# j-wilson/GPflowPILCO

Hardware: AMD Instinct MI355X
Metric: moment_matched_rollout_step_elements_per_sec (higher is better)
Workload: dtype f32; 1 GPU; C3 (BASELINE configs[2]): N=2000 d=8 D=8 H=40 fp32 drift moment-match step / closed rollout; recipe=baseline: BASELINE.md recipe: lengthscales log-U[0.3,3], GP-prior targets, fresh mu~U[0,1]^d / Sigm~; N=2000, d=8, D=8, H=40, B_per_gpu=256, B_total=256, B_this_rank=256, parallelism=dp1 over B (weak), recipe=baseline, steps_requested=418, diag_pairs=f64, offdiag_pairs=f32

## Files before the change

### gpflowpilco_amd/csrc/mm_common.h

```cpp
#pragma once
#include <stddef.h>
#include <stdint.h>
#include "../../include/gpflowpilco_mm.h"

static inline size_t mm_align_up(size_t x, size_t a) { return (x + a - 1) / a * a; }
static inline int mm_round_up_int(int x, int a) { return (x + a - 1) / a * a; }
static inline size_t mm_elem_size(int dtype) { return dtype == MM_F64 ? 8 : 4; }

#define MM_ISTAGE_NO_ROUTE (1 << 20)
#define MM_ISTAGE_ROUTE (1 << 21)
#define MM_ISTAGE_NO_M56 (1 << 22)
#define MM_ISTAGE_OLD_OFFDIAG (1 << 23)

static inline int mm_num_pairs(int L, int flags) {
  return (flags & MM_FULL_OUTPUT_COV) ? L * (L + 1) / 2 : L;
}

static inline int mm_moment_deg(int d) { return d <= 8 ? 4 : 2; }
static inline long long mm_binom(int n, int k) {
  if (k < 0 || k > n) return 0;
  long long r = 1;
  for (int i = 1; i <= k; ++i) r = r * (n - k + i) / i;
  return r;
}
static inline int mm_mono_count(int n, int d) { return (int)mm_binom(d + n - 1, n); }
static inline int mm_mono_offset(int n, int d) { int o = 0; for (int m = 0; m < n; ++m) o += mm_mono_count(m, d); return o; }
static inline size_t mm_rank_table_entries(int d) {
  const int dk = d <= 8 ? 8 : 32, deg = mm_moment_deg(d);
  size_t n = 0, p = 1;
  for (int k = 1; k <= deg; ++k) { p *= dk; n += p; }
  return n;
}
static inline int mm_moment_cols(int d) { return mm_round_up_int(mm_mono_offset(mm_moment_deg(d) + 1, d), 16); }
static inline int mm_moment56_off5(int d) { return d <= 8 ? mm_round_up_int(mm_mono_count(4, d), 128) : 0; }
static inline int mm_moment56_off6(int d) { return d <= 8 ? mm_moment56_off5(d) + mm_round_up_int(mm_mono_count(5, d), 128) : 0; }
static inline int mm_moment56_cols(int d) { return d <= 8 ? mm_moment56_off6(d) + mm_round_up_int(mm_mono_count(6, d), 128) : 0; }
struct MMTab56 { int ins[6], last[6], n_i16, mult2, mult3, n_f32; size_t bytes; };
static inline MMTab56 mm_tab56(int d) {
  MMTab56 t;
  int o = 0;
  for (int m = 0; m < 6; ++m) { t.ins[m] = o; o += mm_mono_count(m, d) * 8; }
  for (int k = 0; k < 6; ++k) { t.last[k] = o; o += mm_mono_count(k, d); }
  t.n_i16 = mm_round_up_int(o, 8);
  t.mult2 = 0; t.mult3 = mm_mono_count(2, d); t.n_f32 = mm_mono_count(2, d) + mm_mono_count(3, d);
  t.bytes = (size_t)t.n_i16 * 2 + (size_t)t.n_f32 * 4;
  return t;
}

struct MMModelLayout {
  int Mp, Kz, nd8, KMp;
  size_t Z64;
  size_t Zt64;
  size_t zbar;
  size_t ls2;
  size_t var;
  size_t meanc;
  size_t beta64;
  size_t Zc64;
  size_t Zc;
  size_t Zs3;
  size_t Zm;
  size_t zmax2;
  size_t rtab;
  size_t Zq2;
  size_t Zm56;
  size_t tab56;
  size_t perm;
  size_t skey;
  size_t zt2;
  size_t Cm;
  size_t total;
};
#define MM_SORT_MIN_M 256

static inline MMModelLayout mm_model_layout(int L, int M, int d, int dtype, int with_C) {
  MMModelLayout o;
  const size_t es = mm_elem_size(dtype), A = 256;
  o.Mp = mm_round_up_int(M, MM_M_ALIGN);
  o.Kz = mm_round_up_int(d, 2);
  o.nd8 = (d + 7) / 8;
  o.KMp = mm_moment_cols(d);
  size_t off = 0;
  o.Z64 = off;    off = mm_align_up(off + (size_t)L * M * d * 8, A);
  o.Zt64 = off;   off = mm_align_up(off + (size_t)L * d * o.Mp * 8, A);
  o.zbar = off;   off = mm_align_up(off + (size_t)L * d * 8, A);
  o.ls2 = off;    off = mm_align_up(off + (size_t)L * d * 8, A);
  o.var = off;    off = mm_align_up(off + (size_t)L * 8, A);
  o.meanc = off;  off = mm_align_up(off + (size_t)L * 8, A);
  o.beta64 = off; off = mm_align_up(off + (size_t)L * M * 8, A);
  o.Zc64 = off;   off = mm_align_up(off + (size_t)L * o.Mp * o.Kz * 8, A);
  o.Zc = o.Zc64;
  if (dtype != MM_F64) { o.Zc = off; off = mm_align_up(off + (size_t)L * o.Mp * o.Kz * es, A); }
  o.Zs3 = off;
  if (dtype != MM_F64) off = mm_align_up(off + (size_t)L * o.Mp * 24 * o.nd8 * 2, A);
  o.Zm = off;
// ... 173 lines not shown
```

### gpflowpilco_amd/csrc/mm_moments.hip

```cpp
#include <hip/hip_runtime.h>
#include <math.h>
#include "mm_common.h"
#include "mm_mono.h"

typedef double f64x4m __attribute__((ext_vector_type(4)));

#define MM_GEMM_RB 64
#define MM_GEMM_NB 128
#define MM_GEMM_KB 32
#define MM_GEMM_AS 34
#define MM_GEMM_BS 144

__device__ __forceinline__ void mm_decode_pair_m(int p, int L, int& a, int& a2) {
  int r = p - L, i = 0;
  while (r >= L - 1 - i) { r -= L - 1 - i; ++i; }
  a = i; a2 = i + 1 + r;
}

__global__ __launch_bounds__(256) __attribute__((amdgpu_waves_per_eu(2, 2))) void k_wmom_gemm(const double* __restrict__ whR, const double* __restrict__ whC,
                                                      const double* __restrict__ Zm, int KMp, int L, int Mp, int B, int Po,
                                                      int nrb, int ncb, int nwork, int col_deg3,
                                                      const unsigned int* __restrict__ amaxc, const double* __restrict__ zmax2,
                                                      const int* __restrict__ gperm, double* __restrict__ mom) {
  const int orig = blockIdx.x;
// ... 235 lines not shown
    const int dsz = 1 << (LB * n);
    const int offn = n == 1 ? off1 : n == 2 ? off2 : n == 3 ? off3 : off4;
    const short* rtn = rtab + (((1 << (LB * n)) - DK) / (DK - 1));
    for (int idx = tid; idx < dsz; idx += 256) {
      const int r = rtn[idx];
      T[MM_PADI(idx)] = r >= 0 ? qh[offn + r] : 0.0;
    }
    __syncthreads();
    for (int t = 0; t < n; ++t) {
      const int sh = LB * t, nfib = dsz >> LB;
      for (int f = tid; f < nfib; f += 256) {
        const int lo = f & ((1 << sh) - 1), hi = f >> sh;
        const int base = (hi << (sh + LB)) + lo;
        double v[DK];
#pragma unroll
        for (int l = 0; l < DK; ++l) v[l] = T[MM_PADI(base + (l << sh))];
        if constexpr (DK == 8) {
#pragma unroll
          for (int k = 0; k < 8; ++k) {
            double s = 0.0;
#pragma unroll
            for (int l = 0; l < 8; ++l) s = fma(Gr[k * 8 + l], v[l], s);
            T[MM_PADI(base + (k << sh))] = s;
          }
        } else {
#pragma unroll 2
          for (int k = 0; k < DK; ++k) {
            double s = 0.0;
#pragma unroll
            for (int l = 0; l < DK; ++l) s = fma(Gs[k * DK + l], v[l], s);
            T[MM_PADI(base + (k << sh))] = s;
          }
        }
      }
      __syncthreads();
    }
    double* cur = T;
    double* oth = U;
    int ksz = dsz;
    double sign_binom = 1.0;
    for (int k = n; k >= 0; --k) {
      const int offk = k == 0 ? 0 : k == 1 ? off1 : k == 2 ? off2 : k == 3 ? off3 : off4;
      double part = 0.0;
      const short* rtk = rtab + (k ? (((1 << (LB * k)) - DK) / (DK - 1)) : 0);
      for (int idx = tid; idx < ksz; idx += 256) {
        const int r = k ? rtk[idx] : 0;
        if (r >= 0) part = fma(cur[MM_PADI(idx)], nh[offk + r], part);
      }
      total = fma(an * sign_binom, part, total);
      if (k == 0) break;
      const int nsz = ksz >> LB;
      for (int idx = tid; idx < nsz; idx += 256) {
        double s = 0.0;
#pragma unroll
        for (int l = 0; l < DK; ++l) s = fma(cur[MM_PADI(l * nsz + idx)], dmu[l], s);
        oth[MM_PADI(idx)] = s;
      }
      __syncthreads();
      double* tsw = cur; cur = oth; oth = tsw;
      ksz = nsz;
      sign_binom = -sign_binom * (double)k / (double)(n - k + 1);
    }
    __syncthreads();
  }
  const double tot = mm_block_sum256m(total, red);
  if (tid == 0) s12[(size_t)b * Po + po] = tot + nh[0] * qh[0];
#undef MM_PADI
}

int mm_launch_wmom_full(const char* packed, const MMModelLayout& ml, char* ws, const MMWorkspaceLayout& wl,
                        int B, int L, int d, hipStream_t stream) {
  const int nrb = ((L - 1) * B + MM_GEMM_RB - 1) / MM_GEMM_RB, ncb = (ml.KMp + MM_GEMM_NB - 1) / MM_GEMM_NB;
  const long long nwork_ll = (long long)L * ncb * MM_MOM_SPLIT * nrb;
  if (nwork_ll <= 0 || nwork_ll > 0x7fffffffLL) return MM_E_DIM;
  hipLaunchKernelGGL(k_wmom_gemm, dim3((int)nwork_ll), dim3(256), 0, stream, (const double*)(ws + wl.whR),
                     (const double*)(ws + wl.whC), (const double*)(packed + ml.Zm), ml.KMp, L, wl.Mp, B, wl.Po, nrb, ncb,
                     (int)nwork_ll, 0x7fffffff , (const unsigned int*)nullptr, (const double*)(packed + ml.zmax2),
                     (const int*)nullptr, (double*)(ws + wl.mom));
  hipError_t e = hipGetLastError();
  return e == hipSuccess ? 0 : (int)e;
}

int mm_launch_moments56(const char* packed, const MMModelLayout& ml, char* ws, const MMWorkspaceLayout& wl,
                        int B, int L, int d, int allow, hipStream_t stream);

int mm_launch_moments(const char* packed, const MMModelLayout& ml, char* ws, const MMWorkspaceLayout& wl,
                      int B, int L, int d, const void* mu_f32, int flags, hipStream_t stream) {
  const double* Zm = (const double*)(packed + ml.Zm);
  double* mom = (double*)(ws + wl.mom);
  const int deg = mm_moment_deg(d) >= 4 ? 3 : mm_moment_deg(d);
  const int ncol_fwd = mm_mono_offset(deg + 1, d);
  const int nrb = ((L - 1) * B + MM_GEMM_RB - 1) / MM_GEMM_RB, ncb = (ncol_fwd + MM_GEMM_NB - 1) / MM_GEMM_NB;
  const long long nwork_ll = (long long)L * ncb * MM_MOM_SPLIT * nrb;
  if (nwork_ll <= 0 || nwork_ll > 0x7fffffffLL) return MM_E_DIM;
  const int nwork = (int)nwork_ll;
  const int allow = (flags & (MM_FORCE_WORST_TIER | MM_ISTAGE_NO_M56)) ? 0 : 1;
  const int col_deg3 = mm_mono_offset(3, d);
  const bool some = allow && mm_moment_deg(d) >= 4;
  if (some) {
    hipLaunchKernelGGL(k_wmom_perm, dim3(L), dim3(1024), 0, stream, (const unsigned int*)(ws + wl.amaxc),
                       (const double*)(packed + ml.zmax2), L, B, wl.Po, (int*)(ws + wl.gperm));
    hipError_t ep = hipGetLastError();
    if (ep != hipSuccess) return (int)ep;
  }
  hipLaunchKernelGGL(k_wmom_gemm, dim3(nwork), dim3(256), 0, stream, (const double*)(ws + wl.whR),
                     (const double*)(ws + wl.whC), Zm, ml.KMp, L, wl.Mp, B, wl.Po, nrb, ncb, nwork, col_deg3,
                     some ? (const unsigned int*)(ws + wl.amaxc) : (const unsigned int*)nullptr,
                     (const double*)(packed + ml.zmax2), some ? (const int*)(ws + wl.gperm) : (const int*)nullptr, mom);
  hipError_t e = hipGetLastError();
  if (e != hipSuccess) return (int)e;
  const int off1 = mm_mono_offset(1, d), off2 = mm_mono_offset(2, d), off3 = mm_mono_offset(3, d), off4 = mm_mono_offset(4, d);
#define MM_SPOLY(DK_, LB_)                                                                                                       \
  do {                                                                                                                          \
    const int dn_ = 1 << (LB_ * deg);                                                                                           \
    const int up_ = dn_ >> LB_;                                                                                                 \
    const size_t shm_ = (size_t)(dn_ + (dn_ >> 5) + up_ + (up_ >> 5) + 2 * ml.KMp + DK_ * DK_ + DK_ + 8) * sizeof(double);      \
    hipLaunchKernelGGL((k_spoly<DK_, LB_>), dim3(wl.Po, B), dim3(256), shm_, stream, (const double*)mom, ml.KMp,                \
                       (const double*)(ws + wl.pairmat), (const double*)(packed + ml.zbar), (const double*)(packed + ml.zmax2), \
                       (const unsigned int*)(ws + wl.amax), (const unsigned int*)(ws + wl.amaxc), (const float*)mu_f32, L, d, wl.P, deg, allow, off1, off2, off3, off4, \
                       (const short*)(packed + ml.rtab),                                                                        \
                       (double)MM_C6_C0, (double)MM_C6_C1, (double*)(ws + wl.s12));                                             \
  } while (0)
  if (d <= 8) MM_SPOLY(8, 3); else MM_SPOLY(32, 5);
#undef MM_SPOLY
  e = hipGetLastError();
  if (e != hipSuccess) return (int)e;
  if (flags & MM_ISTAGE_NO_M56) {
    if (mm_moment56_cols(d) <= 0 || wl.Po <= 0) return 0;
    const hipError_t em = hipMemsetAsync(ws + wl.s56, 0xFF, (size_t)B * wl.Po * sizeof(double), stream);
    if (em != hipSuccess) return (int)em;
    const hipError_t es = hipMemsetAsync(ws + wl.estS, 0, (size_t)B * wl.Po * sizeof(float), stream);
    return es == hipSuccess ? 0 : (int)es;
  }
  return mm_launch_moments56(packed, ml, ws, wl, B, L, d, some ? 1 : 0, stream);
}

__global__ void k_offdiag_stats(const unsigned int* __restrict__ amax, const double* __restrict__ zmax2,
                                const unsigned char* __restrict__ gflag, int ng, int L, int Po, int n,
                                int32_t* __restrict__ out) {
  const int idx = blockIdx.x * blockDim.x + threadIdx.x;
  bool c = false, in = false, part = false;
  int groups = 0;
  if (idx < n) {
    int a, a2;
    mm_decode_pair_m(L + idx % Po, L, a, a2);
    const float b2 = mm_collapse_bound2(amax[idx], zmax2[a2]);
    c = b2 <= MM_COLLAPSE_BOUND2;
    in = b2 <= MM_INSIDE_BOUND2;
    part = !c && mm_item_collapsed(amax[n + idx]);
    for (int g = 0; g < ng; ++g) groups += gflag[(size_t)idx * ng + g] ? 1 : 0;
  }
  const unsigned long long m = __ballot(c), mi = __ballot(in), mp = __ballot(part);
  if ((threadIdx.x & 63) == 0 && m) atomicAdd(out, (int)__popcll(m));
  if ((threadIdx.x & 63) == 0 && mi) atomicAdd(out + 2, (int)__popcll(mi));
  if ((threadIdx.x & 63) == 0 && mp) atomicAdd(out + 4, (int)__popcll(mp));
#pragma unroll
  for (int off = 32; off > 0; off >>= 1) groups += __shfl_down(groups, off, 64);
  if ((threadIdx.x & 63) == 0 && groups) atomicAdd(out + 5, groups);
  if (idx == 0) out[1] = n;
}

extern "C" int mm_offdiag_stats(const void* packed, size_t packed_bytes, int L, int M, int d, int dtype, int B, int flags,
                                const void* workspace, size_t workspace_bytes, int32_t* out, void* stream) {
  if (!packed || !workspace || !out || L <= 0 || M <= 0 || d <= 0 || d > MM_DMAX || B <= 0) return MM_E_ARG;
  const MMModelLayout ml = mm_model_layout(L, M, d, dtype, 1);
  const MMWorkspaceLayout wl = mm_workspace_layout(B, L, M, d, dtype, flags);
  if (packed_bytes < ml.Cm || workspace_bytes < wl.total) return MM_E_WORKSPACE;
  hipStream_t s = (hipStream_t)stream;
  hipError_t e = hipMemsetAsync(out, 0, 6 * sizeof(int32_t), s);
  if (e != hipSuccess) return (int)e;
  if (dtype == MM_F32 && wl.Po > 0) {
    e = hipMemcpyAsync(out + 3, (const char*)workspace + wl.rcount + 4, sizeof(int32_t), hipMemcpyDeviceToDevice, s);
    if (e != hipSuccess) return (int)e;
  }
  if (dtype != MM_F32 || wl.Po == 0 || mm_moment_deg(d) < 4 || (flags & MM_FORCE_WORST_TIER)) return 0;
  const int n = B * wl.Po;
  hipLaunchKernelGGL(k_offdiag_stats, dim3((n + 255) / 256), dim3(256), 0, s, (const unsigned int*)((const char*)workspace + wl.amax),
                     (const double*)((const char*)packed + ml.zmax2), (const unsigned char*)((const char*)workspace + wl.gflag),
                     wl.Mp / MM_GROUP_ROWS, L, wl.Po, n, out);
  e = hipGetLastError();
  return e == hipSuccess ? 0 : (int)e;
}
```

### gpflowpilco_amd/csrc/mm_moments6.hip

```cpp
#include <hip/hip_runtime.h>
#include <math.h>
#include "mm_common.h"
#include "mm_mono.h"
#include "mm_f32_tile.h"
#include <atomic>
#include <type_traits>

__device__ __forceinline__ void mm6_decode_pair_o(int lp, int L, int& a, int& a2) {
  int r = lp, i = 0;
  while (r >= L - 1 - i) { r -= L - 1 - i; ++i; }
  a = i; a2 = i + 1 + r;
}

__global__ __launch_bounds__(256) void k_pack_zm56(char* packed, MMModelLayout lay, int L, int M, int d, int N56p,
                                                   const double* __restrict__ Z) {
  const int c = blockIdx.x, a = blockIdx.y, tid = threadIdx.x;
  const int n4 = mm_binom_i(d + 3, 4), n5 = mm_binom_i(d + 4, 5), n6 = mm_binom_i(d + 5, 6);
  const int off5 = ((n4 + 127) / 128) * 128;
  const int off6 = off5 + ((n5 + 127) / 128) * 128;
  const double* zbar = (const double*)(packed + lay.zbar) + (size_t)a * d;
  unsigned short* oh = (unsigned short*)(packed + lay.Zm56) + (((size_t)a * 2 + 0) * N56p + c) * lay.Mp;
  unsigned short* om = (unsigned short*)(packed + lay.Zm56) + (((size_t)a * 2 + 1) * N56p + c) * lay.Mp;
  int n = 0, k[6] = {0, 0, 0, 0, 0, 0};
  if (c < n4) { n = 4; mm_mono_unrank(c, 4, k); }
// ... 186 lines not shown
#endif
template <int K, bool TRANSG, int MODE, int NC = MM6_NC, int NW = MM6_WAVES>
__device__ __forceinline__ void mm6_step(const float* __restrict__ Tin, int nJin, int nI, float* __restrict__ Tout, int nJp,
                                         const short* __restrict__ ins, int d, const float (&G)[64], const float* __restrict__ multJ,
                                         int xs, float& acc, int wave, int lane) {
  const int chunks = (nJp + 64 * NC - 1) / (64 * NC);
  auto dots = [&](auto i0c, const float (&v)[NC][8], float (&s)[NC][8]) __attribute__((always_inline)) {
    constexpr int I0 = decltype(i0c)::value;
#pragma unroll
    for (int q = 0; q < NC; ++q)
#pragma unroll
      for (int i = I0; i < 8; ++i) s[q][i] = G[0 * 8 + i] * v[q][0];
#pragma unroll
    for (int j = 1; j < 8; ++j)
#pragma unroll
      for (int q = 0; q < NC; ++q)
#pragma unroll
        for (int i = I0; i < 8; ++i) s[q][i] = fmaf(G[j * 8 + i], v[q][j], s[q][i]);
  };
  auto body = [&](int I, int t, const int (&Jp)[NC], const bool (&jv)[NC], const int (&off)[NC][8], const float (&mj)[NC]) __attribute__((always_inline)) {
    const float* tin = Tin + I * nJin;
    float v[NC][8], s[NC][8];
#pragma unroll
    for (int q = 0; q < NC; ++q)
#pragma unroll
      for (int j = 0; j < 8; ++j) v[q][j] = tin[off[q][j]];
    if (t < 4) dots(std::integral_constant<int, 0>{}, v, s);
    else if (t < 6) dots(std::integral_constant<int, 4>{}, v, s);
    else dots(std::integral_constant<int, 6>{}, v, s);
#pragma unroll
    for (int i = 0; i < 8; ++i) {
      if (i >= t && i < d) {
        const int orow = I + mm_binom_i(i + K, K + 1);
        float m3 = 1.0f;
        if constexpr (MODE == 1 && K == 2) {
          const int a = I - ((t * (t + 1)) >> 1);
          m3 = a == t ? (i == t ? 1.0f : 3.0f) : (i == t ? 3.0f : 6.0f);
        } else if constexpr (MODE == 1 && K == 1) {
          m3 = i == t ? 1.0f : 2.0f;
        }
#pragma unroll
        for (int q = 0; q < NC; ++q) {
          if constexpr (MODE == 0) { if (jv[q]) Tout[orow * nJp + Jp[q]] = s[q][i]; }
          else if constexpr (MODE == 1) { if (jv[q]) Tout[orow * xs + Jp[q]] = (m3 * mj[q]) * s[q][i]; }
          else { if (jv[q]) acc = fmaf(s[q][i], Tout[Jp[q] * xs + orow], acc); }
        }
      }
    }
  };
  const int nunit = chunks * nI;
  const float rnI = 1.0f / (float)nI;
  int cprev = -1, off[NC][8], Jc[NC];
  bool jv[NC];
  float mj[NC];
#pragma unroll
  for (int q = 0; q < NC; ++q) { Jc[q] = 0; jv[q] = false; mj[q] = 0.0f; }
  for (int u = wave; u < nunit; u += NW) {
    int c = K == 0 ? u : (int)(((float)u + 0.5f) * rnI);
    c = __builtin_amdgcn_readfirstlane(c);
    const int I = K == 0 ? 0 : __builtin_amdgcn_readfirstlane(u - c * nI);
    if (c != cprev) {
      cprev = c;
#pragma unroll
      for (int q = 0; q < NC; ++q) {
        const int Jp = (c * NC + q) * 64 + lane;
        jv[q] = Jp < nJp;
        Jc[q] = jv[q] ? Jp : nJp - 1;
        const short4 ia = *reinterpret_cast<const short4*>(ins + (size_t)Jc[q] * 8);
        const short4 ib = *reinterpret_cast<const short4*>(ins + (size_t)Jc[q] * 8 + 4);
        off[q][0] = ia.x; off[q][1] = ia.y; off[q][2] = ia.z; off[q][3] = ia.w;
        off[q][4] = ib.x; off[q][5] = ib.y; off[q][6] = ib.z; off[q][7] = ib.w;
        if constexpr (MODE == 1) mj[q] = multJ[Jc[q]];
      }
    }
    int t = 0;
    if constexpr (K > 0) {
#pragma unroll
      for (int q = 1; q < 8; ++q) t += (I >= mm_binom_i(q + K - 1, K)) ? 1 : 0;
    }
    if (jv[0]) body(I, t, Jc, jv, off, mj);
  }
}

__global__ __launch_bounds__(256) void k_item_classes(const unsigned int* __restrict__ amaxc, const double* __restrict__ zmax2,
                                                      int L, int Po, int n, int allow, int* __restrict__ ilist,
                                                      double* __restrict__ s56, float* __restrict__ estS) {
  const int idx = blockIdx.x * 256 + threadIdx.x, lane = threadIdx.x & 63;
  int cls = 3;
  if (idx < n) {
    int a, a2;
    mm6_decode_pair_o(idx % Po, L, a, a2);
    const unsigned int ac = amaxc[idx];
    const float x2 = mm_collapse_bound2(ac, zmax2[a2]);
    cls = (!allow || !mm_item_collapsed(ac)) ? 3 : (x2 > MM_C6_X5_2 ? 0 : (x2 > MM_C6_X4_2 ? 1 : 2));
    if (cls == 3) { s56[idx] = 0.0; estS[idx] = 0.0f; }
  }
  const unsigned long long b01 = __ballot(cls == 0 || cls == 1), b2 = __ballot(cls == 2);
  int base01 = 0, base2 = 0;
  if (lane == 0) {
    if (b01) base01 = atomicAdd(ilist + 0, (int)__popcll(b01));
    if (b2) base2 = atomicAdd(ilist + 2, (int)__popcll(b2));
  }
  base01 = __shfl(base01, 0, 64); base2 = __shfl(base2, 0, 64);
  const unsigned long long below = (1ull << lane) - 1ull;
  if (cls == 0 || cls == 1) ilist[4 + base01 + __popcll(b01 & below)] = idx;
  if (cls == 2) ilist[4 + n - 1 - (base2 + __popcll(b2 & below))] = idx;
}

__device__ __forceinline__ float mm6_estS(float bound2, bool need5, bool need6, double r2, double c2) {
  const double X = sqrt((double)bound2), X3 = X * X * X;
  double amp = fmin(1.0, 64.0 * X3);
  if (!need6) amp += (double)MM_C6_C3 * X3 * X3 / 5.8e-10;
  if (!need5) amp += (double)MM_C6_C2 * X3 * X * X / 5.8e-10;
  return (float)fmin((double)MM_C6_SYS2 * (amp * amp) * r2 * c2, 3.0e38);
}

__global__ __launch_bounds__(MM6_THREADS) void k_spoly56(const float* __restrict__ mom56, int N56p, const double* __restrict__ pairmat,
                                                 const double* __restrict__ zmax2, const unsigned int* __restrict__ amaxc,
                                                 const unsigned char* __restrict__ gflag,
                                                 const double* __restrict__ whR, const double* __restrict__ whC,
                                                 const char* __restrict__ tab, MMTab56 tb, int L, int d, int P, int Mp,
                                                 const int* __restrict__ ilist,
                                                 double* __restrict__ s56, float* __restrict__ estS) {
  extern __shared__ __align__(16) float sm6[];
  const int tid = threadIdx.x;
  const int wave = __builtin_amdgcn_readfirstlane(tid >> 6), lane = tid & 63;
  const int Po = P - L;
  const int nitems = __builtin_amdgcn_readfirstlane(ilist[0]);
  for (int li = blockIdx.x; li < nitems; li += gridDim.x) {
  const size_t item = (size_t)__builtin_amdgcn_readfirstlane(ilist[4 + li]);
  const int b = (int)(item / Po), po = (int)(item - (size_t)b * Po);
  int a, a2;
  mm6_decode_pair_o(po, L, a, a2);
  const float bound2 = mm_collapse_bound2(amaxc[item], zmax2[a2]);
  int sy[7];
#pragma unroll
  for (int k = 0; k < 7; ++k) sy[k] = mm_binom_i(d + k - 1, k);
  const int n56 = sy[4] + sy[5] + sy[6];
  const int off5 = ((sy[4] + 127) / 128) * 128;
  const int off6 = off5 + ((sy[5] + 127) / 128) * 128;
  const bool need5 = bound2 > MM_C6_X4_2, need6 = bound2 > MM_C6_X5_2;
  const int xs = sy[3] + 1;
  float* nq = sm6;
  float* X = nq + 2 * n56;
  float* A = X + sy[3] * xs;
  float* Bf = A + sy[2] * sy[4];
  float* red = sm6 + ((2 * n56 + sy[3] * xs + sy[2] * sy[4] + sy[1] * sy[5] + 1) & ~1);
  for (int idx = tid; idx < 2 * n56; idx += MM6_THREADS) {
    const int side = idx >= n56, c = idx - side * n56;
    const int dg = c < sy[4] ? 4 : (c < sy[4] + sy[5] ? 5 : 6);
    const int col = dg == 4 ? c : (dg == 5 ? off5 + (c - sy[4]) : off6 + (c - sy[4] - sy[5]));
    float v = 0.0f;
    if (dg == 4 || (dg == 5 ? need5 : need6)) v = mom56[(item * 2 + side) * N56p + col];
    nq[idx] = v;
  }
  float* Gl = sm6 + ((2 * n56 + sy[3] * xs + sy[2] * sy[4] + sy[1] * sy[5] + 6 * MM6_WAVES + 2 + 3) & ~3);
  float* Bf4 = Gl + 128;
  float* X4 = Bf4 + sy[1] * sy[3];
  if (tid < 64) {
    const int i = tid >> 3, j = tid & 7;
    const double* pm = pairmat + ((size_t)b * P + (L + po)) * (d * d + 1);
    const float g = (i < d && j < d) ? (float)pm[i * d + j] : 0.0f;
    Gl[tid] = g;
    Gl[64 + j * 8 + i] = g;
  }
  double s2r = 0.0, s2c = 0.0;
  {
    const double* hr = whR + item * Mp;
    const double* hc = whC + item * Mp;
    const unsigned char* gf = gflag + item * (size_t)(Mp / MM_GROUP_ROWS);
    for (int m = tid; m < Mp; m += MM6_THREADS) {
      const double x = gf[m >> 6] ? hr[m] : 0.0, y = hc[m];
      s2r = fma(x, x, s2r); s2c = fma(y, y, s2c);
    }
  }
  __syncthreads();
  float G[64];
  auto load_G = [&](int transposed) __attribute__((always_inline)) {
#pragma unroll
    for (int q = 0; q < 16; ++q) {
      const float4 g4 = *reinterpret_cast<const float4*>(Gl + 64 * transposed + 4 * q);
      G[4 * q] = g4.x; G[4 * q + 1] = g4.y; G[4 * q + 2] = g4.z; G[4 * q + 3] = g4.w;
    }
  };
  const short* tabi = (const short*)tab;
  const float* mult2 = (const float*)(tab + (size_t)tb.n_i16 * 2) + tb.mult2;
  const float* mult3 = (const float*)(tab + (size_t)tb.n_i16 * 2) + tb.mult3;
  float acc5 = 0.0f, acc6 = 0.0f, dummy = 0.0f;
  if (need6) {
    const float* Q6 = nq + n56 + sy[4] + sy[5];
    const float* N6 = nq + sy[4] + sy[5];
    load_G(1);
    mm6_step<0, false, 0>(Q6, sy[6], 1, Bf, sy[5], tabi + tb.ins[5], d, G, nullptr, 0, dummy, wave, lane);
    __syncthreads();
    mm6_step<1, false, 0>(Bf, sy[5], sy[1], A, sy[4], tabi + tb.ins[4], d, G, nullptr, 0, dummy, wave, lane);
    __syncthreads();
    mm6_step<2, false, 1>(A, sy[4], sy[2], X, sy[3], tabi + tb.ins[3], d, G, mult3, xs, dummy, wave, lane);
    __syncthreads();
    load_G(0);
    mm6_step<0, true, 0>(N6, sy[6], 1, Bf, sy[5], tabi + tb.ins[5], d, G, nullptr, 0, dummy, wave, lane);
    __syncthreads();
    mm6_step<1, true, 0>(Bf, sy[5], sy[1], A, sy[4], tabi + tb.ins[4], d, G, nullptr, 0, dummy, wave, lane);
    __syncthreads();
    mm6_step<2, true, 2>(A, sy[4], sy[2], X, sy[3], tabi + tb.ins[3], d, G, nullptr, xs, acc6, wave, lane);
    __syncthreads();
  }
  float acc4 = 0.0f;
  {
    const float* Q5 = nq + n56 + sy[4];
    const float* N5 = nq + sy[4];
    const float* Q4 = nq + n56;
    const float* N4 = nq;
    const int xs4 = sy[2] + 1;
    load_G(1);
    if (need5) mm6_step<0, false, 0>(Q5, sy[5], 1, Bf, sy[4], tabi + tb.ins[4], d, G, nullptr, 0, dummy, wave, lane);
    mm6_step<0, false, 0>(Q4, sy[4], 1, Bf4, sy[3], tabi + tb.ins[3], d, G, nullptr, 0, dummy, wave, lane);
    __syncthreads();
    if (need5) mm6_step<1, false, 0>(Bf, sy[4], sy[1], A, sy[3], tabi + tb.ins[3], d, G, nullptr, 0, dummy, wave, lane);
    mm6_step<1, false, 1, 1>(Bf4, sy[3], sy[1], X4, sy[2], tabi + tb.ins[2], d, G, mult2, xs4, dummy, wave, lane);
    __syncthreads();
    if (need5) {
      mm6_step<2, false, 1, 1>(A, sy[3], sy[2], X, sy[2], tabi + tb.ins[2], d, G, mult2, xs, dummy, wave, lane);
      __syncthreads();
    }
    load_G(0);
    if (need5) mm6_step<0, true, 0>(N5, sy[5], 1, Bf, sy[4], tabi + tb.ins[4], d, G, nullptr, 0, dummy, wave, lane);
    mm6_step<0, true, 0>(N4, sy[4], 1, Bf4, sy[3], tabi + tb.ins[3], d, G, nullptr, 0, dummy, wave, lane);
    __syncthreads();
    if (need5) mm6_step<1, true, 2>(Bf, sy[4], sy[1], X, sy[3], tabi + tb.ins[3], d, G, nullptr, xs, acc5, wave, lane);
    mm6_step<1, true, 2, 1>(Bf4, sy[3], sy[1], X4, sy[2], tabi + tb.ins[2], d, G, nullptr, xs4, acc4, wave, lane);
  }
  double tot = (double)MM_C6_C1 * (double)acc4 + (double)MM_C6_C2 * (double)acc5 + (double)MM_C6_C3 * (double)acc6;
#pragma unroll
  for (int off = 32; off > 0; off >>= 1) {
    tot += __shfl_down(tot, off, 64); s2r += __shfl_down(s2r, off, 64); s2c += __shfl_down(s2c, off, 64);
  }
  double* redd = reinterpret_cast<double*>(red);
  if (lane == 0) { redd[wave * 3 + 0] = tot; redd[wave * 3 + 1] = s2r; redd[wave * 3 + 2] = s2c; }
  __syncthreads();
  if (tid == 0) {
    double t = 0.0, r2 = 0.0, c2 = 0.0;
    for (int w = 0; w < MM6_WAVES; ++w) { t += redd[w * 3]; r2 += redd[w * 3 + 1]; c2 += redd[w * 3 + 2]; }
    s56[item] = t;
    estS[item] = mm6_estS(bound2, need5, need6, r2, c2);
  }
  __syncthreads();
  }
}

__global__ __launch_bounds__(256) void k_spoly4(const float* __restrict__ mom56, int N56p, const double* __restrict__ pairmat,
                                                const double* __restrict__ zmax2, const unsigned int* __restrict__ amaxc,
                                                const unsigned char* __restrict__ gflag,
                                                const double* __restrict__ whR, const double* __restrict__ whC,
                                                const char* __restrict__ tab, MMTab56 tb, int L, int d, int P, int Mp, int ntotal,
                                                const int* __restrict__ ilist,
                                                double* __restrict__ s56, float* __restrict__ estS) {
  extern __shared__ __align__(16) float sm4[];
  constexpr int NW = 4;
  const int tid = threadIdx.x;
  const int wave = __builtin_amdgcn_readfirstlane(tid >> 6), lane = tid & 63;
  const int Po = P - L;
  int sy[5];
#pragma unroll
  for (int k = 0; k < 5; ++k) sy[k] = mm_binom_i(d + k - 1, k);
  const int xs4 = sy[2] + 1;
  float* nq = sm4;
  float* Bf4 = nq + 2 * sy[4];
  float* X4 = Bf4 + sy[1] * sy[3];
  float* Gl = sm4 + ((2 * sy[4] + sy[1] * sy[3] + sy[2] * xs4 + 3) & ~3);
  double* redd = reinterpret_cast<double*>(Gl + 128);
  const short* tabi = (const short*)tab;
  const float* mult2 = (const float*)(tab + (size_t)tb.n_i16 * 2) + tb.mult2;
  const int nitems = __builtin_amdgcn_readfirstlane(ilist[2]);
  for (int li = blockIdx.x; li < nitems; li += gridDim.x) {
    const size_t item = (size_t)__builtin_amdgcn_readfirstlane(ilist[4 + ntotal - 1 - li]);
    const int b = (int)(item / Po), po = (int)(item - (size_t)b * Po);
    int a, a2;
    mm6_decode_pair_o(po, L, a, a2);
    const float bound2 = mm_collapse_bound2(amaxc[item], zmax2[a2]);
    for (int idx = tid; idx < 2 * sy[4]; idx += 256) {
      const int side = idx >= sy[4], c = idx - side * sy[4];
      nq[idx] = mom56[(item * 2 + side) * N56p + c];
    }
    if (tid < 64) {
      const int i = tid >> 3, j = tid & 7;
      const double* pm = pairmat + ((size_t)b * P + (L + po)) * (d * d + 1);
      const float g = (i < d && j < d) ? (float)pm[i * d + j] : 0.0f;
      Gl[tid] = g;
      Gl[64 + j * 8 + i] = g;
    }
    double s2r = 0.0, s2c = 0.0;
    {
      const double* hr = whR + item * Mp;
      const double* hc = whC + item * Mp;
      const unsigned char* gf = gflag + item * (size_t)(Mp / MM_GROUP_ROWS);
      for (int m = tid; m < Mp; m += 256) {
        const double x = gf[m >> 6] ? hr[m] : 0.0, y = hc[m];
        s2r = fma(x, x, s2r); s2c = fma(y, y, s2c);
      }
    }
    __syncthreads();
    float G[64];
    auto load_G = [&](int transposed) __attribute__((always_inline)) {
#pragma unroll
      for (int q = 0; q < 16; ++q) {
        const float4 g4 = *reinterpret_cast<const float4*>(Gl + 64 * transposed + 4 * q);
        G[4 * q] = g4.x; G[4 * q + 1] = g4.y; G[4 * q + 2] = g4.z; G[4 * q + 3] = g4.w;
      }
    };
    float acc4 = 0.0f, dummy = 0.0f;
    const float* Q4 = nq + sy[4];
    const float* N4 = nq;
    load_G(1);
    mm6_step<0, false, 0, MM6_NC, NW>(Q4, sy[4], 1, Bf4, sy[3], tabi + tb.ins[3], d, G, nullptr, 0, dummy, wave, lane);
    __syncthreads();
    mm6_step<1, false, 1, 1, NW>(Bf4, sy[3], sy[1], X4, sy[2], tabi + tb.ins[2], d, G, mult2, xs4, dummy, wave, lane);
    __syncthreads();
    load_G(0);
    mm6_step<0, true, 0, MM6_NC, NW>(N4, sy[4], 1, Bf4, sy[3], tabi + tb.ins[3], d, G, nullptr, 0, dummy, wave, lane);
    __syncthreads();
    mm6_step<1, true, 2, 1, NW>(Bf4, sy[3], sy[1], X4, sy[2], tabi + tb.ins[2], d, G, nullptr, xs4, acc4, wave, lane);
    double tot = (double)MM_C6_C1 * (double)acc4;
#pragma unroll
    for (int off = 32; off > 0; off >>= 1) {
      tot += __shfl_down(tot, off, 64); s2r += __shfl_down(s2r, off, 64); s2c += __shfl_down(s2c, off, 64);
    }
    if (lane == 0) { redd[wave * 3 + 0] = tot; redd[wave * 3 + 1] = s2r; redd[wave * 3 + 2] = s2c; }
    __syncthreads();
    if (tid == 0) {
      double t = 0.0, r2 = 0.0, c2 = 0.0;
      for (int w = 0; w < NW; ++w) { t += redd[w * 3]; r2 += redd[w * 3 + 1]; c2 += redd[w * 3 + 2]; }
      s56[item] = t;
      estS[item] = mm6_estS(bound2, false, false, r2, c2);
    }
    __syncthreads();
  }
}

int mm_launch_moments56(const char* packed, const MMModelLayout& ml, char* ws, const MMWorkspaceLayout& wl,
                        int B, int L, int d, int allow, hipStream_t stream) {
  const int N56p = mm_moment56_cols(d);
  if (N56p <= 0 || wl.Po <= 0) return 0;
  if (allow) {
    const int nrb = ((L - 1) * B + MM6_TB - 1) / MM6_TB, ncb = N56p / MM6_TB;
    const long long nwork_ll = (long long)L * ncb * nrb;
    if (nwork_ll <= 0 || nwork_ll > 0x7fffffffLL) return MM_E_DIM;
    if ((size_t)B * wl.Po * 4 * wl.Mp >= 0xffffffffull || (size_t)L * 2 * N56p * wl.Mp >= 0xffffffffull) return MM_E_DIM;
    const size_t shm = 2 * MM6_STAGE_BYTES + MM6_TB * sizeof(int);
    static std::atomic<unsigned long long> attr_done{0ull};
    int dev = 0;
    if (hipGetDevice(&dev) != hipSuccess) dev = 64;
    const unsigned long long bit = (dev >= 0 && dev < 64) ? (1ull << dev) : 0ull;
    if (!bit || !(attr_done.load() & bit)) {
      const hipError_t ea = hipFuncSetAttribute((const void*)k_wmom56_gemm, hipFuncAttributeMaxDynamicSharedMemorySize, (int)shm);
      if (ea != hipSuccess) return (int)ea;
      attr_done.fetch_or(bit);
    }
    hipLaunchKernelGGL(k_wmom56_gemm, dim3((int)nwork_ll), dim3(256), shm, stream, (const unsigned short*)(ws + wl.wsp),
                       (const unsigned short*)(packed + ml.Zm56), N56p, L, wl.Mp, B, wl.Po, nrb, ncb, (int)nwork_ll,
                       mm_moment56_off5(d) / MM6_TB, mm_moment56_off6(d) / MM6_TB,
                       (const int*)(ws + wl.gperm), (float*)(ws + wl.mom56));
    hipError_t e = hipGetLastError();
    if (e != hipSuccess) return (int)e;
  }
  const int nitem = B * wl.Po;
  int* ilist = (int*)(ws + wl.ilist);
  {
    const hipError_t em = hipMemsetAsync(ilist, 0, 16, stream);
    if (em != hipSuccess) return (int)em;
  }
  hipLaunchKernelGGL(k_item_classes, dim3((nitem + 255) / 256), dim3(256), 0, stream, (const unsigned int*)(ws + wl.amaxc),
                     (const double*)(packed + ml.zmax2), L, wl.Po, nitem, allow, ilist, (double*)(ws + wl.s56), (float*)(ws + wl.estS));
  {
    const hipError_t ec = hipGetLastError();
    if (ec != hipSuccess) return (int)ec;
  }
  if (!allow) return 0;
  int sy[7];
  for (int k = 0; k < 7; ++k) sy[k] = mm_mono_count(k, d);
  size_t nfl = (size_t)2 * (sy[4] + sy[5] + sy[6]) + (size_t)sy[3] * (sy[3] + 1) + (size_t)sy[2] * sy[4] + (size_t)sy[1] * sy[5] + 6 * MM6_WAVES + 128 + 16
               + (size_t)sy[1] * sy[3] + (size_t)sy[2] * (sy[2] + 1);
  nfl = (nfl + 1) & ~(size_t)1;
  const size_t shm = nfl * sizeof(float);
  static std::atomic<unsigned long long> attr2_done{0ull};
  static std::atomic<int> ncu_cached[64];
  int dev = 0;
  if (hipGetDevice(&dev) != hipSuccess) dev = 64;
  const unsigned long long bit2 = (dev >= 0 && dev < 64) ? (1ull << dev) : 0ull;
  int ncu = bit2 ? ncu_cached[dev].load() : 0;
  if (!bit2 || !(attr2_done.load() & bit2)) {
    const hipError_t ea = hipFuncSetAttribute((const void*)k_spoly56, hipFuncAttributeMaxDynamicSharedMemorySize, 160 * 1024);
    if (ea != hipSuccess) return (int)ea;
    int v = 0;
    if (hipDeviceGetAttribute(&v, hipDeviceAttributeMultiprocessorCount, dev < 64 ? dev : 0) != hipSuccess || v <= 0) v = 256;
    ncu = v;
    if (bit2) { ncu_cached[dev].store(v); attr2_done.fetch_or(bit2); }
  }
  if (ncu <= 0) ncu = 256;
  const int g56 = nitem < ncu ? nitem : ncu, g4 = nitem < 8 * ncu ? nitem : 8 * ncu;
  hipLaunchKernelGGL(k_spoly56, dim3(g56), dim3(MM6_THREADS), shm, stream, (const float*)(ws + wl.mom56), N56p,
                     (const double*)(ws + wl.pairmat), (const double*)(packed + ml.zmax2), (const unsigned int*)(ws + wl.amaxc),
                     (const unsigned char*)(ws + wl.gflag), (const double*)(ws + wl.whR), (const double*)(ws + wl.whC),
                     packed + ml.tab56, mm_tab56(d), L, d, wl.P, wl.Mp, (const int*)ilist, (double*)(ws + wl.s56), (float*)(ws + wl.estS));
  {
    const hipError_t e5 = hipGetLastError();
    if (e5 != hipSuccess) return (int)e5;
  }
  const size_t shm4 = (size_t)(((2 * sy[4] + sy[1] * sy[3] + sy[2] * (sy[2] + 1) + 3) & ~3) + 128 + 2 * 3 * 4 + 8) * sizeof(float);
  hipLaunchKernelGGL(k_spoly4, dim3(g4), dim3(256), shm4, stream, (const float*)(ws + wl.mom56), N56p,
                     (const double*)(ws + wl.pairmat), (const double*)(packed + ml.zmax2), (const unsigned int*)(ws + wl.amaxc),
                     (const unsigned char*)(ws + wl.gflag), (const double*)(ws + wl.whR), (const double*)(ws + wl.whC),
                     packed + ml.tab56, mm_tab56(d), L, d, wl.P, wl.Mp, nitem, (const int*)ilist, (double*)(ws + wl.s56),
                     (float*)(ws + wl.estS));
  hipError_t e = hipGetLastError();
  return e == hipSuccess ? 0 : (int)e;
}
```

Baseline: 40400 rollout step-elements/s (B*H per rollout second).

## Add d=8 compile-time specialized symmetric-tensor contraction steps for spoly56/spoly4

Adds a templated mm6_step8 path for d=8 in which symmetric-tensor sizes, strides and row offsets are compile-time constants. It uses packed float2 FMAs and explicit LDS address-space pointers, and splits the index range into four unrolled branches. The k_spoly56 and k_spoly4 kernels become templated on D8 and dispatch to this path when d==8, with a new flag to fall back to the old generic step. This targets index arithmetic and LDS-access overhead in the degree-5/6 moment polynomial contraction, at the cost of larger code, more register pressure and more template instantiations.

After: 42400 rollout step-elements/s (B*H per rollout second) (median of 6 runs). +5.0%, better.

```diff
diff --git a/gpflowpilco_amd/csrc/mm_common.h b/gpflowpilco_amd/csrc/mm_common.h
--- a/gpflowpilco_amd/csrc/mm_common.h
+++ b/gpflowpilco_amd/csrc/mm_common.h
@@ -11,6 +11,7 @@
 #define MM_ISTAGE_ROUTE (1 << 21)
 #define MM_ISTAGE_NO_M56 (1 << 22)
 #define MM_ISTAGE_OLD_OFFDIAG (1 << 23)
+#define MM_ISTAGE_OLD_SPOLY56 (1 << 24)
 
 static inline int mm_num_pairs(int L, int flags) {
   return (flags & MM_FULL_OUTPUT_COV) ? L * (L + 1) / 2 : L;
diff --git a/gpflowpilco_amd/csrc/mm_moments.hip b/gpflowpilco_amd/csrc/mm_moments.hip
--- a/gpflowpilco_amd/csrc/mm_moments.hip
+++ b/gpflowpilco_amd/csrc/mm_moments.hip
@@ -341,7 +341,7 @@
 }
 
 int mm_launch_moments56(const char* packed, const MMModelLayout& ml, char* ws, const MMWorkspaceLayout& wl,
-                        int B, int L, int d, int allow, hipStream_t stream);
+                        int B, int L, int d, int allow, int old_spoly56, hipStream_t stream);
 
 int mm_launch_moments(const char* packed, const MMModelLayout& ml, char* ws, const MMWorkspaceLayout& wl,
                       int B, int L, int d, const void* mu_f32, int flags, hipStream_t stream) {
@@ -391,7 +391,7 @@
     const hipError_t es = hipMemsetAsync(ws + wl.estS, 0, (size_t)B * wl.Po * sizeof(float), stream);
     return es == hipSuccess ? 0 : (int)es;
   }
-  return mm_launch_moments56(packed, ml, ws, wl, B, L, d, some ? 1 : 0, stream);
+  return mm_launch_moments56(packed, ml, ws, wl, B, L, d, some ? 1 : 0, (flags & MM_ISTAGE_OLD_SPOLY56) ? 1 : 0, stream);
 }
 
 __global__ void k_offdiag_stats(const unsigned int* __restrict__ amax, const double* __restrict__ zmax2,
diff --git a/gpflowpilco_amd/csrc/mm_moments6.hip b/gpflowpilco_amd/csrc/mm_moments6.hip
--- a/gpflowpilco_amd/csrc/mm_moments6.hip
+++ b/gpflowpilco_amd/csrc/mm_moments6.hip
@@ -292,6 +292,171 @@
   }
 }
 
+typedef float mm6_f2 __attribute__((ext_vector_type(2)));
+typedef __attribute__((address_space(3))) float mm6_lds_f;
+constexpr int mm6_cbinom(int n, int k) {
+  if (k < 0 || k > n) return 0;
+  int r = 1;
+  for (int i = 1; i <= k; ++i) r = r * (n - k + i) / i;
+  return r;
+}
+constexpr int mm6_sym8(int k) { return mm6_cbinom(8 + k - 1, k); }
+
+template <int K, int MODE, int NJIN, int NJP, int XS, int NC, int NW>
+__device__ __forceinline__ void mm6_step8(const float* __restrict__ Tin_, float* __restrict__ Tout_, const short* __restrict__ ins,
+                                          const float (&G)[64], const float* __restrict__ multJ, float& acc, int wave, int lane) {
+  asm volatile("" : "+v"(lane));
+  unsigned a_in = (unsigned)(size_t)(const mm6_lds_f*)Tin_, a_out = (unsigned)(size_t)(mm6_lds_f*)Tout_;
+  asm volatile("" : "+s"(a_in));
+  asm volatile("" : "+s"(a_out));
+  const mm6_lds_f* Tin = (const mm6_lds_f*)(size_t)a_in;
+  mm6_lds_f* Tout = (mm6_lds_f*)(size_t)a_out;
+  constexpr int NI = mm6_sym8(K);
+  constexpr int CH = (NJP + 64 * NC - 1) / (64 * NC);
+  constexpr int ST = MODE == 0 ? NJP : XS;
+  static_assert(K >= 0 && K <= 2, "K of the n <= 6 chains");
+  static_assert(mm6_cbinom(7 + K, K + 1) * ST * 4 < 65536, "the row term is a 16-bit ds offset");
+  auto low = [](int t) constexpr { return mm6_cbinom(t + K - 1, K); };
+  auto row = [](int i) constexpr { return mm6_cbinom(i + K, K + 1); };
+  int off[NC][8], Jc[NC];
+  bool jv[NC];
+  float mj[NC];
+  auto load_c = [&](int c) __attribute__((always_inline)) {
+#pragma unroll
+    for (int q = 0; q < NC; ++q) {
+      const int Jp = (c * NC + q) * 64 + lane;
+      jv[q] = Jp < NJP;
+      Jc[q] = jv[q] ? Jp : NJP - 1;
+      const short4 ia = *reinterpret_cast<const short4*>(ins + (size_t)Jc[q] * 8);
+      const short4 ib = *reinterpret_cast<const short4*>(ins + (size_t)Jc[q] * 8 + 4);
+      off[q][0] = ia.x; off[q][1] = ia.y; off[q][2] = ia.z; off[q][3] = ia.w;
+      off[q][4] = ib.x; off[q][5] = ib.y; off[q][6] = ib.z; off[q][7] = ib.w;
+      if constexpr (MODE == 1) mj[q] = multJ[Jc[q]];
+    }
+  };
+  auto body = [&](auto i0c, int I, bool first) __attribute__((always_inline)) {
+    constexpr int I0 = decltype(i0c)::value;
+    const mm6_lds_f* tin = Tin + I * NJIN;
+    float v[NC][8], s[NC][8];
+#pragma unroll
+    for (int q = 0; q < NC; ++q)
+#pragma unroll
+      for (int j = 0; j < 8; ++j) v[q][j] = tin[off[q][j]];
+#pragma unroll
+    for (int q = 0; q < NC; ++q) asm volatile("; unit %c1" : "+v"(v[q][0]) : "n"(I0 * 16 + K * 4 + MODE));
+    mm6_f2 s2[NC][4];
+#pragma unroll
+    for (int q = 0; q < NC; ++q)
+#pragma unroll
+      for (int p = I0 / 2; p < 4; ++p) s2[q][p] = mm6_f2{G[2 * p], G[2 * p + 1]} * mm6_f2{v[q][0], v[q][0]};
+#pragma unroll
+    for (int j = 1; j < 8; ++j)
+#pragma unroll
+      for (int q = 0; q < NC; ++q)
+#pragma unroll
+        for (int p = I0 / 2; p < 4; ++p)
+          s2[q][p] = __builtin_elementwise_fma(mm6_f2{G[j * 8 + 2 * p], G[j * 8 + 2 * p + 1]}, mm6_f2{v[q][j], v[q][j]}, s2[q][p]);
+#pragma unroll
+    for (int q = 0; q < NC; ++q)
+#pragma unroll
+      for (int p = I0 / 2; p < 4; ++p) {
+        asm volatile("" : "+v"(s2[q][p]));
+        s[q][2 * p] = s2[q][p].x; s[q][2 * p + 1] = s2[q][p].y;
+      }
+    if constexpr (MODE == 0) {
+#pragma unroll
+      for (int q = 0; q < NC; ++q) {
+        mm6_lds_f* o = Tout + I * ST + Jc[q];
+        if (jv[q]) {
+          if (first) o[row(I0) * ST] = s[q][I0];
+#pragma unroll
+          for (int i = I0 + 1; i < 8; ++i) o[row(i) * ST] = s[q][i];
+          asm volatile("; stores %c0" : : "n"((I0 * 16 + K * 4 + MODE) * 2 + q));
+        }
+      }
+    } else if constexpr (MODE == 1) {
+      float m_eq = 1.0f, m_gt = 2.0f;
+      if constexpr (K == 2) {
+        const bool aeq = first ? (I - low(I0) == I0) : (I - low(I0 + 1) == I0 + 1);
+        m_eq = aeq ? 1.0f : 3.0f;
+        m_gt = aeq ? 3.0f : 6.0f;
+      }
+      const float m_1 = first ? m_gt : m_eq;
+#pragma unroll
+      for (int q = 0; q < NC; ++q) {
+        mm6_lds_f* o = Tout + I * ST + Jc[q];
+        if (jv[q]) {
+          if (first) o[row(I0) * ST] = (m_eq * mj[q]) * s[q][I0];
+          o[row(I0 + 1) * ST] = (m_1 * mj[q]) * s[q][I0 + 1];
+#pragma unroll
+          for (int i = I0 + 2; i < 8; ++i) o[row(i) * ST] = (m_gt * mj[q]) * s[q][i];
+          asm volatile("; stores %c0" : : "n"((I0 * 16 + K * 4 + MODE) * 2 + q));
+        }
+      }
+    } else {
+      const mm6_lds_f* x[NC];
+#pragma unroll
+      for (int q = 0; q < NC; ++q) x[q] = Tout + Jc[q] * ST + I;
+      if (first) {
+#pragma unroll
+        for (int q = 0; q < NC; ++q) acc = (q == 0 || jv[q]) ? fmaf(s[q][I0], x[q][row(I0)], acc) : acc;
+      }
+#pragma unroll
+      for (int i = I0 + 1; i < 8; ++i)
+#pragma unroll
+        for (int q = 0; q < NC; ++q) acc = (q == 0 || jv[q]) ? fmaf(s[q][i], x[q][row(i)], acc) : acc;
+    }
+    asm volatile("; end %c0" : : "n"(I0 * 16 + K * 4 + MODE));
+  };
+  auto unit = [&](int I) __attribute__((always_inline)) {
+    if constexpr (K == 0) {
+      body(std::integral_constant<int, 0>{}, 0, true);
+    } else {
+      if (I < low(4)) {
+        if (I < low(2)) body(std::integral_constant<int, 0>{}, I, I < low(1));
+        else body(std::integral_constant<int, 2>{}, I, I < low(3));
+      } else {
+        if (I < low(6)) body(std::integral_constant<int, 4>{}, I, I < low(5));
+        else body(std::integral_constant<int, 6>{}, I, I < low(7));
+      }
+    }
+  };
+  if constexpr (CH == 1) {
+    if (wave < NI) {
+      load_c(0);
+      for (int I = wave; I < NI; I += NW)
+        if (jv[0]) unit(I);
+    }
+  } else if constexpr (NI == 1) {
+    for (int c = wave; c < CH; c += NW) {
+      load_c(c);
+      if (jv[0]) unit(0);
+    }
+  } else if constexpr (MODE != 2 && NW % CH == 0) {
+    const int c = wave % CH;
+    load_c(c);
+    for (int I = wave / CH; I < NI; I += NW / CH)
+      if (jv[0]) unit(I);
+  } else {
+    int cprev = -1;
+    for (int u = wave; u < CH * NI; u += NW) {
+      const int c = u / NI, I = u - c * NI;
+      if (c != cprev) { cprev = c; load_c(c); }
+      if (jv[0]) unit(I);
+    }
+  }
+}
+
+template <bool D8, int K, bool TRANSG, int MODE, int NC, int NW, int KIN, int XS8>
+__device__ __forceinline__ void mm6_do(const float* __restrict__ Tin, float* __restrict__ Tout, const int* sy, const short* __restrict__ tabi,
+                                       const MMTab56& tb, int d, const float (&G)[64], const float* __restrict__ multJ, int xs,
+                                       float& acc, int wave, int lane) {
+  if constexpr (D8)
+    mm6_step8<K, MODE, mm6_sym8(KIN), mm6_sym8(KIN - 1), XS8, NC, NW>(Tin, Tout, tabi + tb.ins[KIN - 1], G, multJ, acc, wave, lane);
+  else
+    mm6_step<K, TRANSG, MODE, NC, NW>(Tin, sy[KIN], sy[K], Tout, sy[KIN - 1], tabi + tb.ins[KIN - 1], d, G, multJ, xs, acc, wave, lane);
+}
+
 __global__ __launch_bounds__(256) void k_item_classes(const unsigned int* __restrict__ amaxc, const double* __restrict__ zmax2,
                                                       int L, int Po, int n, int allow, int* __restrict__ ilist,
                                                       double* __restrict__ s56, float* __restrict__ estS) {
@@ -325,14 +490,17 @@
   return (float)fmin((double)MM_C6_SYS2 * (amp * amp) * r2 * c2, 3.0e38);
 }
 
+template <bool D8>
 __global__ __launch_bounds__(MM6_THREADS) void k_spoly56(const float* __restrict__ mom56, int N56p, const double* __restrict__ pairmat,
                                                  const double* __restrict__ zmax2, const unsigned int* __restrict__ amaxc,
                                                  const unsigned char* __restrict__ gflag,
                                                  const double* __restrict__ whR, const double* __restrict__ whC,
-                                                 const char* __restrict__ tab, MMTab56 tb, int L, int d, int P, int Mp,
+                                                 const char* __restrict__ tab, MMTab56 tb, int L, int d_, int P, int Mp,
                                                  const int* __restrict__ ilist,
                                                  double* __restrict__ s56, float* __restrict__ estS) {
   extern __shared__ __align__(16) float sm6[];
+  const int d = D8 ? 8 : d_;
+  constexpr int NW = MM6_WAVES, NC = MM6_NC;
   const int tid = threadIdx.x;
   const int wave = __builtin_amdgcn_readfirstlane(tid >> 6), lane = tid & 63;
   const int Po = P - L;
@@ -401,18 +569,18 @@
     const float* Q6 = nq + n56 + sy[4] + sy[5];
     const float* N6 = nq + sy[4] + sy[5];
     load_G(1);
-    mm6_step<0, false, 0>(Q6, sy[6], 1, Bf, sy[5], tabi + tb.ins[5], d, G, nullptr, 0, dummy, wave, lane);
-    __syncthreads();
-    mm6_step<1, false, 0>(Bf, sy[5], sy[1], A, sy[4], tabi + tb.ins[4], d, G, nullptr, 0, dummy, wave, lane);
-    __syncthreads();
-    mm6_step<2, false, 1>(A, sy[4], sy[2], X, sy[3], tabi + tb.ins[3], d, G, mult3, xs, dummy, wave, lane);
+    mm6_do<D8, 0, false, 0, NC, NW, 6, 0>(Q6, Bf, sy, tabi, tb, d, G, nullptr, 0, dummy, wave, lane);
+    __syncthreads();
+    mm6_do<D8, 1, false, 0, NC, NW, 5, 0>(Bf, A, sy, tabi, tb, d, G, nullptr, 0, dummy, wave, lane);
+    __syncthreads();
+    mm6_do<D8, 2, false, 1, NC, NW, 4, 121>(A, X, sy, tabi, tb, d, G, mult3, xs, dummy, wave, lane);
     __syncthreads();
     load_G(0);
-    mm6_step<0, true, 0>(N6, sy[6], 1, Bf, sy[5], tabi + tb.ins[5], d, G, nullptr, 0, dummy, wave, lane);
-    __syncthreads();
-    mm6_step<1, true, 0>(Bf, sy[5], sy[1], A, sy[4], tabi + tb.ins[4], d, G, nullptr, 0, dummy, wave, lane);
-    __syncthreads();
-    mm6_step<2, true, 2>(A, sy[4], sy[2], X, sy[3], tabi + tb.ins[3], d, G, nullptr, xs, acc6, wave, lane);
+    mm6_do<D8, 0, true, 0, NC, NW, 6, 0>(N6, Bf, sy, tabi, tb, d, G, nullptr, 0, dummy, wave, lane);
+    __syncthreads();
+    mm6_do<D8, 1, true, 0, NC, NW, 5, 0>(Bf, A, sy, tabi, tb, d, G, nullptr, 0, dummy, wave, lane);
+    __syncthreads();
+    mm6_do<D8, 2, true, 2, NC, NW, 4, 121>(A, X, sy, tabi, tb, d, G, nullptr, xs, acc6, wave, lane);
     __syncthreads();
   }
   float acc4 = 0.0f;
@@ -423,22 +591,22 @@
     const float* N4 = nq;
     const int xs4 = sy[2] + 1;
     load_G(1);
-    if (need5) mm6_step<0, false, 0>(Q5, sy[5], 1, Bf, sy[4], tabi + tb.ins[4], d, G, nullptr, 0, dummy, wave, lane);
-    mm6_step<0, false, 0>(Q4, sy[4], 1, Bf4, sy[3], tabi + tb.ins[3], d, G, nullptr, 0, dummy, wave, lane);
-    __syncthreads();
-    if (need5) mm6_step<1, false, 0>(Bf, sy[4], sy[1], A, sy[3], tabi + tb.ins[3], d, G, nullptr, 0, dummy, wave, lane);
-    mm6_step<1, false, 1, 1>(Bf4, sy[3], sy[1], X4, sy[2], tabi + tb.ins[2], d, G, mult2, xs4, dummy, wave, lane);
+    if (need5) mm6_do<D8, 0, false, 0, NC, NW, 5, 0>(Q5, Bf, sy, tabi, tb, d, G, nullptr, 0, dummy, wave, lane);
+    mm6_do<D8, 0, false, 0, NC, NW, 4, 0>(Q4, Bf4, sy, tabi, tb, d, G, nullptr, 0, dummy, wave, lane);
+    __syncthreads();
+    if (need5) mm6_do<D8, 1, false, 0, NC, NW, 4, 0>(Bf, A, sy, tabi, tb, d, G, nullptr, 0, dummy, wave, lane);
+    mm6_do<D8, 1, false, 1, 1, NW, 3, 37>(Bf4, X4, sy, tabi, tb, d, G, mult2, xs4, dummy, wave, lane);
     __syncthreads();
     if (need5) {
-      mm6_step<2, false, 1, 1>(A, sy[3], sy[2], X, sy[2], tabi + tb.ins[2], d, G, mult2, xs, dummy, wave, lane);
+      mm6_do<D8, 2, false, 1, 1, NW, 3, 121>(A, X, sy, tabi, tb, d, G, mult2, xs, dummy, wave, lane);
       __syncthreads();
     }
     load_G(0);
-    if (need5) mm6_step<0, true, 0>(N5, sy[5], 1, Bf, sy[4], tabi + tb.ins[4], d, G, nullptr, 0, dummy, wave, lane);
-    mm6_step<0, true, 0>(N4, sy[4], 1, Bf4, sy[3], tabi + tb.ins[3], d, G, nullptr, 0, dummy, wave, lane);
-    __syncthreads();
-    if (need5) mm6_step<1, true, 2>(Bf, sy[4], sy[1], X, sy[3], tabi + tb.ins[3], d, G, nullptr, xs, acc5, wave, lane);
-    mm6_step<1, true, 2, 1>(Bf4, sy[3], sy[1], X4, sy[2], tabi + tb.ins[2], d, G, nullptr, xs4, acc4, wave, lane);
+    if (need5) mm6_do<D8, 0, true, 0, NC, NW, 5, 0>(N5, Bf, sy, tabi, tb, d, G, nullptr, 0, dummy, wave, lane);
+    mm6_do<D8, 0, true, 0, NC, NW, 4, 0>(N4, Bf4, sy, tabi, tb, d, G, nullptr, 0, dummy, wave, lane);
+    __syncthreads();
+    if (need5) mm6_do<D8, 1, true, 2, NC, NW, 4, 121>(Bf, X, sy, tabi, tb, d, G, nullptr, xs, acc5, wave, lane);
+    mm6_do<D8, 1, true, 2, 1, NW, 3, 37>(Bf4, X4, sy, tabi, tb, d, G, nullptr, xs4, acc4, wave, lane);
   }
   double tot = (double)MM_C6_C1 * (double)acc4 + (double)MM_C6_C2 * (double)acc5 + (double)MM_C6_C3 * (double)acc6;
 #pragma unroll
@@ -458,14 +626,17 @@
   }
 }
 
+template <bool D8>
 __global__ __launch_bounds__(256) void k_spoly4(const float* __restrict__ mom56, int N56p, const double* __restrict__ pairmat,
                                                 const double* __restrict__ zmax2, const unsigned int* __restrict__ amaxc,
                                                 const unsigned char* __restrict__ gflag,
                                                 const double* __restrict__ whR, const double* __restrict__ whC,
-                                                const char* __restrict__ tab, MMTab56 tb, int L, int d, int P, int Mp, int ntotal,
+                                                const char* __restrict__ tab, MMTab56 tb, int L, int d_, int P, int Mp, int ntotal,
                                                 const int* __restrict__ ilist,
                                                 double* __restrict__ s56, float* __restrict__ estS) {
   extern __shared__ __align__(16) float sm4[];
+  const int d = D8 ? 8 : d_;
+  constexpr int NC0 = D8 ? 1 : MM6_NC;
   constexpr int NW = 4;
   const int tid = threadIdx.x;
   const int wave = __builtin_amdgcn_readfirstlane(tid >> 6), lane = tid & 63;
@@ -522,14 +693,14 @@
     const float* Q4 = nq + sy[4];
     const float* N4 = nq;
     load_G(1);
-    mm6_step<0, false, 0, MM6_NC, NW>(Q4, sy[4], 1, Bf4, sy[3], tabi + tb.ins[3], d, G, nullptr, 0, dummy, wave, lane);
-    __syncthreads();
-    mm6_step<1, false, 1, 1, NW>(Bf4, sy[3], sy[1], X4, sy[2], tabi + tb.ins[2], d, G, mult2, xs4, dummy, wave, lane);
+    mm6_do<D8, 0, false, 0, NC0, NW, 4, 0>(Q4, Bf4, sy, tabi, tb, d, G, nullptr, 0, dummy, wave, lane);
+    __syncthreads();
+    mm6_do<D8, 1, false, 1, 1, NW, 3, 37>(Bf4, X4, sy, tabi, tb, d, G, mult2, xs4, dummy, wave, lane);
     __syncthreads();
     load_G(0);
-    mm6_step<0, true, 0, MM6_NC, NW>(N4, sy[4], 1, Bf4, sy[3], tabi + tb.ins[3], d, G, nullptr, 0, dummy, wave, lane);
-    __syncthreads();
-    mm6_step<1, true, 2, 1, NW>(Bf4, sy[3], sy[1], X4, sy[2], tabi + tb.ins[2], d, G, nullptr, xs4, acc4, wave, lane);
+    mm6_do<D8, 0, true, 0, NC0, NW, 4, 0>(N4, Bf4, sy, tabi, tb, d, G, nullptr, 0, dummy, wave, lane);
+    __syncthreads();
+    mm6_do<D8, 1, true, 2, 1, NW, 3, 37>(Bf4, X4, sy, tabi, tb, d, G, nullptr, xs4, acc4, wave, lane);
     double tot = (double)MM_C6_C1 * (double)acc4;
 #pragma unroll
     for (int off = 32; off > 0; off >>= 1) {
@@ -548,7 +719,7 @@
 }
 
 int mm_launch_moments56(const char* packed, const MMModelLayout& ml, char* ws, const MMWorkspaceLayout& wl,
-                        int B, int L, int d, int allow, hipStream_t stream) {
+                        int B, int L, int d, int allow, int old_spoly56, hipStream_t stream) {
   const int N56p = mm_moment56_cols(d);
   if (N56p <= 0 || wl.Po <= 0) return 0;
   if (allow) {
@@ -599,7 +770,8 @@
   const unsigned long long bit2 = (dev >= 0 && dev < 64) ? (1ull << dev) : 0ull;
   int ncu = bit2 ? ncu_cached[dev].load() : 0;
   if (!bit2 || !(attr2_done.load() & bit2)) {
-    const hipError_t ea = hipFuncSetAttribute((const void*)k_spoly56, hipFuncAttributeMaxDynamicSharedMemorySize, 160 * 1024);
+    hipError_t ea = hipFuncSetAttribute((const void*)k_spoly56<false>, hipFuncAttributeMaxDynamicSharedMemorySize, 160 * 1024);
+    if (ea == hipSuccess) ea = hipFuncSetAttribute((const void*)k_spoly56<true>, hipFuncAttributeMaxDynamicSharedMemorySize, 160 * 1024);
     if (ea != hipSuccess) return (int)ea;
     int v = 0;
     if (hipDeviceGetAttribute(&v, hipDeviceAttributeMultiprocessorCount, dev < 64 ? dev : 0) != hipSuccess || v <= 0) v = 256;
@@ -608,7 +780,8 @@
   }
   if (ncu <= 0) ncu = 256;
   const int g56 = nitem < ncu ? nitem : ncu, g4 = nitem < 8 * ncu ? nitem : 8 * ncu;
-  hipLaunchKernelGGL(k_spoly56, dim3(g56), dim3(MM6_THREADS), shm, stream, (const float*)(ws + wl.mom56), N56p,
+  const bool d8 = d == 8 && !old_spoly56;
+  hipLaunchKernelGGL((d8 ? k_spoly56<true> : k_spoly56<false>), dim3(g56), dim3(MM6_THREADS), shm, stream, (const float*)(ws + wl.mom56), N56p,
                      (const double*)(ws + wl.pairmat), (const double*)(packed + ml.zmax2), (const unsigned int*)(ws + wl.amaxc),
                      (const unsigned char*)(ws + wl.gflag), (const double*)(ws + wl.whR), (const double*)(ws + wl.whC),
                      packed + ml.tab56, mm_tab56(d), L, d, wl.P, wl.Mp, (const int*)ilist, (double*)(ws + wl.s56), (float*)(ws + wl.estS));
@@ -617,7 +790,7 @@
     if (e5 != hipSuccess) return (int)e5;
   }
   const size_t shm4 = (size_t)(((2 * sy[4] + sy[1] * sy[3] + sy[2] * (sy[2] + 1) + 3) & ~3) + 128 + 2 * 3 * 4 + 8) * sizeof(float);
-  hipLaunchKernelGGL(k_spoly4, dim3(g4), dim3(256), shm4, stream, (const float*)(ws + wl.mom56), N56p,
+  hipLaunchKernelGGL((d8 ? k_spoly4<true> : k_spoly4<false>), dim3(g4), dim3(256), shm4, stream, (const float*)(ws + wl.mom56), N56p,
                      (const double*)(ws + wl.pairmat), (const double*)(packed + ml.zmax2), (const unsigned int*)(ws + wl.amaxc),
                      (const unsigned char*)(ws + wl.gflag), (const double*)(ws + wl.whR), (const double*)(ws + wl.whC),
                      packed + ml.tab56, mm_tab56(d), L, d, wl.P, wl.Mp, nitem, (const int*)ilist, (double*)(ws + wl.s56),
```
